# mohammadasim98/mv-ldm

Measured on AMD Instinct MI355X. Metric: denoised views/sec @ 256x256, 4 views, 50 DDIM steps, higher is better.
Workload: dtype bf16

## Files before the change

mv_ldm_amd/_build.py:

```python
from __future__ import annotations

import json
import os
import re
import subprocess
import sys
from concurrent.futures import ThreadPoolExecutor
from pathlib import Path

CSRC = Path(__file__).resolve().parent / "csrc"
LIB = CSRC / "libmvldm_hip.so"
SOURCES = ["api.cpp", "plan.cpp", "igemm.hip", "igemm_small.hip", "igemm_large.hip", "igemm_xl.hip", "igemm_halo.hip", "pack.hip", "attention.hip", "norm.hip", "misc.hip",
           "wgrad.hip", "attention_bwd.hip", "norm_bwd.hip", "train_misc.hip", "linear_pp.hip", "linear_pw.hip", "linear_ws.hip", "linear_rs.hip", "skinny.hip", "metrics.hip"]
HEADERS = [*sorted(CSRC.glob("*.h")), CSRC.parent.parent / "include" / "mvldm.h"]
FLAGS = ["--offload-arch=gfx950", "-O3", "-std=c++17", "-fPIC", "-ffp-contract=off", "-Wno-unused-result",
         "-Rpass-analysis=kernel-resource-usage"]
RES = CSRC / "kernel_resources.json"


def _hipcc() -> str:
    for c in (os.environ.get("HIPCC"), "/opt/rocm/bin/hipcc", "hipcc"):
        if c and (os.path.isabs(c) and os.path.exists(c) or not os.path.isabs(c)):
            return c
    raise RuntimeError("hipcc not found")


def _stale(target: Path, deps) -> bool:
    if not target.exists():
        return True
    t = target.stat().st_mtime
    return any(Path(d).stat().st_mtime > t for d in deps)


def build(force: bool = False, verbose: bool = False) -> Path:
    hipcc = _hipcc()
    flags = list(FLAGS)
    if os.environ.get("MVLDM_EXPERIMENTS") == "1":
        flags.append("-DMVLDM_EXPERIMENTS")
    objs, jobs = [], []
    for src in SOURCES:
        s = CSRC / src
        o = CSRC / (s.stem + ".o")
        objs.append(o)
        if force or _stale(o, [s, *HEADERS]):
            cmd = [hipcc, *flags, "-x", "hip", "-c", str(s), "-o", str(o)]
            jobs.append(cmd)
    if jobs:
        def run(cmd):
            if verbose:
                print(" ".join(cmd), flush=True)
            r = subprocess.run(cmd, capture_output=True, text=True)
            if r.returncode:
                raise RuntimeError(f"hipcc failed: {' '.join(cmd)}\n{r.stdout}\n{r.stderr}")
            Path(cmd[-1]).with_suffix(".res.json").write_text(json.dumps(_resources(r.stderr), indent=0))
        with ThreadPoolExecutor(max_workers=min(8, len(jobs))) as ex:
            list(ex.map(run, jobs))
    if force or jobs or _stale(LIB, objs):
        cmd = [hipcc, "--offload-arch=gfx950", "-shared", "-fPIC", "-o", str(LIB), *map(str, objs)]
        r = subprocess.run(cmd, capture_output=True, text=True)
        if r.returncode:
            raise RuntimeError(f"link failed:\n{r.stdout}\n{r.stderr}")
    parts = [o.with_suffix(".res.json") for o in objs]
    if all(q.exists() for q in parts) and (not RES.exists() or _stale(RES, parts)):
        merged = {}
        for q in parts:
            merged.update(json.loads(q.read_text()))
        RES.write_text(json.dumps(merged, indent=0, sort_keys=True))
    return LIB


_FIELDS = {"VGPRs": "vgpr", "AGPRs": "agpr", "TotalSGPRs": "sgpr", "ScratchSize [bytes/lane]": "scratch", "VGPRs Spill": "vgpr_spill",
           "Occupancy [waves/SIMD]": "waves_per_simd"}


def _resources(stderr: str) -> dict:
    out, cur = {}, None
    for line in stderr.splitlines():
        m = re.search(r"remark:\s+(.*?)\s*\[-Rpass-analysis", line)
        if not m:
            continue
        body = m.group(1)
        if body.startswith("Function Name:"):
            cur = out.setdefault(body.split(":", 1)[1].strip(), {})
        elif cur is not None and ":" in body:
            k, v = body.rsplit(":", 1)
            if k.strip() in _FIELDS and v.strip().lstrip("-").isdigit():
                cur[_FIELDS[k.strip()]] = int(v)
    return out


if __name__ == "__main__":
    print(build(force="--force" in sys.argv, verbose=True))
```

mv_ldm_amd/csrc/attention.hip:

```cpp
#include <algorithm>
#include <cstdlib>

#include "common.h"

namespace mvldm {

struct AttnParams {
    const void* q; const void* k; const void* v; void* out;
    const int32_t* seg;
    int ld_q, ld_k, ld_v, ld_o, heads, d;
    float scale_log2e;
    int nqt;
    int remap;
    float* lse;
    int lse_ld;
};

template <typename T> struct AttnMma;
typedef __attribute__((ext_vector_type(4))) __bf16 bf16x4_t;
typedef __attribute__((ext_vector_type(4))) _Float16 f16x4_t;
template <> struct AttnMma<bf16_t> {
    using Frag = bf16x8;
    using Half = bf16x4_t;
    static __device__ __forceinline__ Half tr_read(const bf16_t* p) {
// ... 258 lines not shown
#pragma unroll
                    for (int r = 0; r < 16; ++r) {
                        const int key = kb * 32 + (r & 3) + 8 * (r >> 2) + 4 * hi;
                        o[0][db] = __builtin_amdgcn_mfma_f32_32x32x2f32(vrow[key], s[0][kb][r], o[0][db], 0, 0, 0);
                    }
            }
        } else {
            const int gi = lane >> 4, sl = lane & 15;
            const T* vsrc = Vt + (4 * (gi >> 1) + (sl >> 2)) * VP + (gi & 1) * 16 + 4 * (sl & 3);
            auto pv = [&](const int qb) {
#pragma unroll
                for (int db = 0; db < NDB; ++db) {
#pragma unroll
                    for (int ks = 0; ks < 4; ++ks) {
                        const T* pa = vsrc + (ks * 16) * VP + db * 32;
                        const auto lo = AttnMma<T>::tr_read(pa);
                        const auto up = AttnMma<T>::tr_read(pa + 8 * VP);
                        const typename AttnMma<T>::Frag a = __builtin_shufflevector(lo, up, 0, 1, 2, 3, 4, 5, 6, 7);
                        o[qb][db] = AttnMma<T>::mma(a, pf[qb][ks], o[qb][db]);
                    }
                }
            };
            if constexpr (QB == 1) {
                sm_max(0);
                sm_exp(0);
                pv(0);
            } else {
                sm_max(0);
                sm_exp(0);
                sm_max(1);
                __builtin_amdgcn_sched_barrier(0);
                pv(0);
                sm_exp(1);
#pragma unroll
                for (int g = 0; g < NDB * 4; ++g) {
                    __builtin_amdgcn_sched_group_barrier(0x100, 2, 0);
                    __builtin_amdgcn_sched_group_barrier(0x008, 1, 0);
                    __builtin_amdgcn_sched_group_barrier(0x002, (96 + NDB * 4 - 1) / (NDB * 4), 0);
                }
                __builtin_amdgcn_sched_barrier(0);
                pv(1);
            }
        }
        __syncthreads();
    }

#pragma unroll
    for (int qb = 0; qb < QB; ++qb) {
        float l_tot;
        if constexpr (ONES) {
            l_tot = 0.f;
#pragma unroll
            for (int db = 0; db < NDB; ++db)
#pragma unroll
                for (int q8 = 0; q8 < 4; ++q8)
                    if (db * 32 + q8 * 8 == d) l_tot = o[qb][db][4 * q8];
        } else {
            l_tot = l_run[qb] + __shfl_xor(l_run[qb], 32, 64);
        }
        const float inv = l_tot > 0.f ? 1.0f / l_tot : 0.f;
        if (!q_ok[qb]) continue;
        if (p.lse && hi == 0) p.lse[(size_t)head * p.lse_ld + q_row0 + q_local[qb]] = m_run[qb] * p.scale_log2e + __log2f(l_tot);
        T* op = reinterpret_cast<T*>(p.out) + (size_t)(q_row0 + q_local[qb]) * p.ld_o + head * d;
#pragma unroll
        for (int db = 0; db < NDB; ++db)
#pragma unroll
            for (int r4 = 0; r4 < 4; ++r4) {
                const int dd = db * 32 + 8 * r4 + 4 * hi;
                if (dd < d) {
                    if constexpr (F32) {
                        f32x4 w = {o[qb][db][r4 * 4 + 0] * inv, o[qb][db][r4 * 4 + 1] * inv, o[qb][db][r4 * 4 + 2] * inv, o[qb][db][r4 * 4 + 3] * inv};
                        *reinterpret_cast<f32x4*>(op + dd) = w;
                    } else {
                        union { T e[4]; u32x2 raw; } w;
#pragma unroll
                        for (int e = 0; e < 4; ++e) w.e[e] = from_f32<T>(o[qb][db][r4 * 4 + e] * inv);
                        *reinterpret_cast<u32x2*>(op + dd) = w.raw;
                    }
                }
            }
    }
}


template <typename T, int NCH>
__global__ __launch_bounds__(256) void attention_wide_kernel(const AttnParams p) {
    constexpr int EPC = Elt<T>::EPC;
    const int lane = threadIdx.x & 63, wave = threadIdx.x >> 6;
    const int head = blockIdx.y;
    const int4 sg = reinterpret_cast<const int4*>(p.seg)[blockIdx.z];
    const int q_row0 = sg.x, q_len = sg.y, kv_row0 = sg.z, kv_len = sg.w;
    const int q_local = blockIdx.x * 4 + wave;
    if (q_local >= q_len) return;
    const int d = p.d, nch = d / EPC;
    const T* qp = reinterpret_cast<const T*>(p.q) + (size_t)(q_row0 + q_local) * p.ld_q + head * d;
    float qv[NCH][EPC], ov[NCH][EPC];
#pragma unroll
    for (int j = 0; j < NCH; ++j) {
        const int ch = lane + 64 * j;
        Chunk<T> c;
        if (ch < nch) c = load_chunk<T>(qp + ch * EPC); else c.zero();
#pragma unroll
        for (int i = 0; i < EPC; ++i) { qv[j][i] = c.get(i) * p.scale_log2e; ov[j][i] = 0.f; }
    }
    const T* kb = reinterpret_cast<const T*>(p.k) + (size_t)kv_row0 * p.ld_k + head * d;
    const T* vb = reinterpret_cast<const T*>(p.v) + (size_t)kv_row0 * p.ld_v + head * d;
    float m_run = -INFINITY, l_run = 0.f;
    for (int key = 0; key < kv_len; ++key) {
        float part = 0.f;
        Chunk<T> vc[NCH];
#pragma unroll
        for (int j = 0; j < NCH; ++j) {
            const int ch = lane + 64 * j;
            Chunk<T> kc;
            if (ch < nch) {
                kc = load_chunk<T>(kb + (size_t)key * p.ld_k + ch * EPC);
                vc[j] = load_chunk<T>(vb + (size_t)key * p.ld_v + ch * EPC);
            } else {
                kc.zero();
                vc[j].zero();
            }
#pragma unroll
            for (int i = 0; i < EPC; ++i) part += qv[j][i] * kc.get(i);
        }
        const float sv = wave_sum(part);
        const float m_new = fmaxf(m_run, sv);
        const float alpha = exp2f(m_run - m_new), pv = exp2f(sv - m_new);
        m_run = m_new;
        l_run = l_run * alpha + pv;
#pragma unroll
        for (int j = 0; j < NCH; ++j)
#pragma unroll
            for (int i = 0; i < EPC; ++i) ov[j][i] = ov[j][i] * alpha + pv * vc[j].get(i);
    }
    const float inv = l_run > 0.f ? 1.0f / l_run : 0.f;
    T* op = reinterpret_cast<T*>(p.out) + (size_t)(q_row0 + q_local) * p.ld_o + head * d;
#pragma unroll
    for (int j = 0; j < NCH; ++j) {
        const int ch = lane + 64 * j;
        if (ch < nch) {
            Chunk<T> c;
#pragma unroll
            for (int i = 0; i < EPC; ++i) c.set(i, ov[j][i] * inv);
            store_chunk<T>(op + ch * EPC, c);
        }
    }
}

constexpr int BKW = 32;
template <typename T, int DSL>
__global__ __launch_bounds__(256, 2)
void attention_dsplit_kernel(const AttnParams p) {
    static_assert(sizeof(T) == 2 && DSL % 32 == 0 && DSL <= 128, "d-split attention: 16-bit, slices of 32..128 columns");
    using Frag = typename AttnMma<T>::Frag;
    constexpr int EPC = 8, D = 4 * DSL;
    constexpr int NDB = DSL / 32, NQ = DSL / 16;
    constexpr int KP = D + 8, VP = v_pitch(D);
    constexpr int NCH = D / EPC;
    constexpr int NST = BKW * NCH / 256;
    static_assert(BKW * NCH % 256 == 0, "whole chunks per thread");
    extern __shared__ __attribute__((aligned(16))) char smem[];
    T* Ks = reinterpret_cast<T*>(smem);
    T* Vt = Ks + BKW * KP;
    float* Xs = reinterpret_cast<float*>(Vt + BKW * VP);

    const int tid = threadIdx.x, lane = tid & 63;
// ... 117 lines not shown
        l_run += rs;
        Frag pf[2];
#pragma unroll
        for (int ks = 0; ks < 2; ++ks)
#pragma unroll
            for (int j = 0; j < 8; ++j) pf[ks][j] = from_f32<T>(s[ks * 8 + j]);
#pragma unroll
        for (int db = 0; db < NDB; ++db)
#pragma unroll
            for (int ks = 0; ks < 2; ++ks) {
                const T* pa = vsrc + (ks * 16) * VP + db * 32;
                const auto lo = AttnMma<T>::tr_read(pa);
                const auto up = AttnMma<T>::tr_read(pa + 8 * VP);
                const Frag a = __builtin_shufflevector(lo, up, 0, 1, 2, 3, 4, 5, 6, 7);
                o[db] = AttnMma<T>::mma(a, pf[ks], o[db]);
            }
        __syncthreads();
    }
    const float l_tot = l_run + __shfl_xor(l_run, 32, 64);
    const float inv = l_tot > 0.f ? 1.0f / l_tot : 0.f;
    if (!q_ok) return;
    T* op = reinterpret_cast<T*>(p.out) + (size_t)(q_row0 + q_local) * p.ld_o + head * D + dsl0;
#pragma unroll
    for (int db = 0; db < NDB; ++db)
#pragma unroll
        for (int r4 = 0; r4 < 4; ++r4) {
            union { T e[4]; u32x2 raw; } w;
#pragma unroll
            for (int e = 0; e < 4; ++e) w.e[e] = from_f32<T>(o[db][r4 * 4 + e] * inv);
            *reinterpret_cast<u32x2*>(op + db * 32 + 8 * r4 + 4 * hi) = w.raw;
        }
}

template <typename T, int DSL> static int launch_attn_dsplit(AttnParams p, int n_seg, int max_q_len, hipStream_t s) {
    constexpr int D = 4 * DSL;
    constexpr int smem = (BKW * (D + 8) + BKW * v_pitch(D)) * 2 + 4 * 64 * 16 * 4;
    auto kern = attention_dsplit_kernel<T, DSL>;
    static std::atomic<uint64_t> attr_done{0};
    if (int rc0 = ensure_dyn_smem(reinterpret_cast<const void*>(kern), smem, attr_done)) return rc0;
    p.nqt = (max_q_len + 31) / 32;
    p.remap = 1;
    hipLaunchKernelGGL(kern, dim3(p.nqt * p.heads * n_seg), dim3(256), smem, s, p);
    return check_launch();
}

template <typename T> static int launch_attn_wide(const AttnParams& p, int n_seg, int max_q_len, hipStream_t s) {
    const int nch = p.d / Elt<T>::EPC;
    dim3 grid((max_q_len + 3) / 4, p.heads, n_seg);
    if (nch <= 64) hipLaunchKernelGGL((attention_wide_kernel<T, 1>), grid, dim3(256), 0, s, p);
    else if (nch <= 128) hipLaunchKernelGGL((attention_wide_kernel<T, 2>), grid, dim3(256), 0, s, p);
    else if (nch <= 256) hipLaunchKernelGGL((attention_wide_kernel<T, 4>), grid, dim3(256), 0, s, p);
    else return set_error(MVLDM_ERR_UNSUPPORTED, "attention: head_dim %d too wide", p.d);
    return check_launch();
}

static const int kEnvAttnQB = knob_int("MVLDM_ATTN_QB", 1);

template <typename T, int DP, bool ONES, int QB> static int launch_attn_k(AttnParams p, int n_seg, int max_q_len, hipStream_t s) {
    constexpr bool F32 = std::is_same<T, float>::value;
    constexpr int DV = (DP + 31) / 32 * 32;
    constexpr int KP = F32 ? (DP + 1) : (DP + 8);
    constexpr int VP = F32 ? (BKV + 1) : v_pitch(DV);
    constexpr int smem = (BKV * KP + (F32 ? DV * VP : BKV * VP)) * (int)sizeof(T);
    auto kern = attention_kernel<T, DP, ONES, QB>;
    static std::atomic<uint64_t> attr_done{0};
    if (int rc0 = ensure_dyn_smem(reinterpret_cast<const void*>(kern), smem, attr_done)) return rc0;
    p.nqt = (max_q_len + BQ * QB - 1) / (BQ * QB);
    p.remap = max_q_len <= 2048;
    dim3 grid(p.nqt * p.heads * n_seg);
    hipLaunchKernelGGL(kern, grid, dim3(256), smem, s, p);
    return check_launch();
}

template <typename T, int DP, bool ONES> static int launch_attn_q(AttnParams p, int n_seg, int max_q_len, hipStream_t s) {
    if constexpr (sizeof(T) == 2 && DP <= 64) {
        const long wgs2 = (long)((max_q_len + 2 * BQ - 1) / (2 * BQ)) * p.heads * n_seg;
        if (kEnvAttnQB == 2 && max_q_len >= 2 * BQ && wgs2 >= 512) return launch_attn_k<T, DP, ONES, 2>(p, n_seg, max_q_len, s);
    }
    return launch_attn_k<T, DP, ONES, 1>(p, n_seg, max_q_len, s);
}

template <typename T, int DP> static int launch_attn(AttnParams p, int n_seg, int max_q_len, hipStream_t s) {
    if constexpr (sizeof(T) == 2) {
        if (p.d % 8 == 0 && p.d < DP) return launch_attn_q<T, DP, true>(p, n_seg, max_q_len, s);
    }
    return launch_attn_q<T, DP, false>(p, n_seg, max_q_len, s);
}

int attention_run(const void* q, const void* k, const void* v, void* out, int ld_q, int ld_k, int ld_v, int ld_o,
                  int heads, int head_dim, const int32_t* seg, int n_seg, int max_q_len, float scale, int dtype,
                  float* lse, int lse_ld, hipStream_t s) {
    const int epc = dtype == MVLDM_F32 ? 4 : 8;
    MVLDM_REQUIRE(head_dim > 0 && head_dim % epc == 0, "attention: head_dim %d must be a multiple of %d", head_dim, epc);
    if (n_seg == 0 || max_q_len == 0) return MVLDM_OK;
    MVLDM_REQUIRE(q && k && v && out && seg, "attention: null pointer");
    MVLDM_REQUIRE(ld_q % epc == 0 && ld_k % epc == 0 && ld_v % epc == 0 && ld_o % 4 == 0, "attention: row strides must keep 16-byte alignment");
    if (n_seg == 0 || max_q_len == 0) return MVLDM_OK;
    MVLDM_REQUIRE(!lse || head_dim <= 160, "attention: log-sum-exp output only on the MFMA kernels (head_dim <= 160)");
    AttnParams p{q, k, v, out, seg, ld_q, ld_k, ld_v, ld_o, heads, head_dim, scale * 1.4426950408889634f, 0, 0, lse, lse_ld};
    const int dp = (head_dim + 15) / 16 * 16;
    return dispatch_dtype(dtype, [&](auto t) {
        using T = decltype(t);
        if (head_dim > 160) {
            if constexpr (sizeof(T) == 2) {
                static const bool valu = knob_int("MVLDM_ATTN_WIDE_VALU", 0) != 0;
                if (head_dim == 512 && !valu && !p.lse) return launch_attn_dsplit<T, 128>(p, n_seg, max_q_len, s);
            }
            return launch_attn_wide<T>(p, n_seg, max_q_len, s);
        }
        switch (dp) {
            case 16: return launch_attn<T, 16>(p, n_seg, max_q_len, s);
            case 32: return launch_attn<T, 32>(p, n_seg, max_q_len, s);
            case 48: return launch_attn<T, 48>(p, n_seg, max_q_len, s);
            case 64: return launch_attn<T, 64>(p, n_seg, max_q_len, s);
            case 80: return launch_attn<T, 80>(p, n_seg, max_q_len, s);
            case 96: return launch_attn<T, 96>(p, n_seg, max_q_len, s);
            case 112: return launch_attn<T, 112>(p, n_seg, max_q_len, s);
            case 128: return launch_attn<T, 128>(p, n_seg, max_q_len, s);
            case 144: return launch_attn<T, 144>(p, n_seg, max_q_len, s);
            case 160: return launch_attn<T, 160>(p, n_seg, max_q_len, s);
            default: return set_error(MVLDM_ERR_UNSUPPORTED, "attention: head_dim %d", head_dim);
        }
    });
}

template <typename T>
__global__ __launch_bounds__(256) void attn_merge_kernel(const T* __restrict__ oa, const float* __restrict__ lse_a, const T* __restrict__ ob,
                                                         const float* __restrict__ lse_b, T* __restrict__ out, const int32_t* __restrict__ a_img,
                                                         const int32_t* __restrict__ b_img, const int32_t* __restrict__ out_img, int n_img, int tokens,
                                                         int heads, int d, int ld_a, int ld_b, int ld_o, int lla, int llb) {
    constexpr int EPC = Elt<T>::EPC;
    const int cpr = heads * d / EPC;
    const size_t total = (size_t)n_img * tokens * cpr;
    for (size_t i = (size_t)blockIdx.x * 256 + threadIdx.x; i < total; i += (size_t)gridDim.x * 256) {
        const int c = (int)(i % cpr);
        const size_t rt = i / cpr;
        const int t = (int)(rt % tokens), k = (int)(rt / tokens);
        const size_t ra = (size_t)a_img[k] * tokens + t, rb = (size_t)b_img[k] * tokens + t, ro = (size_t)out_img[k] * tokens + t;
        const int head = c * EPC / d;
        const float la = lse_a[(size_t)head * lla + ra], lb = lse_b[(size_t)head * llb + rb];
        const float mx = fmaxf(la, lb);
        const float ea = __builtin_amdgcn_exp2f(la - mx), eb = __builtin_amdgcn_exp2f(lb - mx);
        const float inv = 1.0f / (ea + eb);
        const float wa = ea * inv, wb = eb * inv;
        const Chunk<T> va = load_chunk<T>(oa + ra * ld_a + c * EPC), vb = load_chunk<T>(ob + rb * ld_b + c * EPC);
        Chunk<T> o;
#pragma unroll
        for (int e = 0; e < EPC; ++e) o.set(e, va.get(e) * wa + vb.get(e) * wb);
        store_chunk<T>(out + ro * ld_o + c * EPC, o);
    }
}

int attention_merge_run(const void* oa, const float* lse_a, const void* ob, const float* lse_b, void* out, const int32_t* a_img,
                        const int32_t* b_img, const int32_t* out_img, int n_img, int tokens, int heads, int head_dim, int ld_a, int ld_b,
                        int ld_o, int lse_ld_a, int lse_ld_b, int dtype, hipStream_t s) {
    const int epc = dtype == MVLDM_F32 ? 4 : 8;
    if (n_img == 0 || tokens == 0) return MVLDM_OK;
    MVLDM_REQUIRE(oa && ob && out && lse_a && lse_b && a_img && b_img && out_img, "attention_merge: null pointer");
    MVLDM_REQUIRE(head_dim % epc == 0 && ld_a % epc == 0 && ld_b % epc == 0 && ld_o % epc == 0, "attention_merge: 16-byte alignment");
    const size_t total = (size_t)n_img * tokens * (heads * head_dim / epc);
    return dispatch_dtype(dtype, [&](auto t) {
        using T = decltype(t);
        hipLaunchKernelGGL(attn_merge_kernel<T>, dim3((unsigned)std::min<size_t>((total + 255) / 256, 16384)), dim3(256), 0, s, reinterpret_cast<const T*>(oa),
                           lse_a, reinterpret_cast<const T*>(ob), lse_b, reinterpret_cast<T*>(out), a_img, b_img, out_img, n_img, tokens, heads, head_dim,
                           ld_a, ld_b, ld_o, lse_ld_a, lse_ld_b);
        return check_launch();
// ... 18 lines not shown
```

mv_ldm_amd/csrc/igemm.hip:

```cpp
#include <algorithm>
#include <cstdio>
#include <cstdlib>

#include "igemm_common.h"

namespace mvldm {

template <typename T> __global__ __launch_bounds__(256) void igemm_splitk_reduce(const IgemmParams p) {
    const bool geglu = p.epilogue == MVLDM_EPI_GEGLU;
    const size_t total = (size_t)p.M * p.n_dst;
    const size_t slab = (size_t)p.M * p.n_pad;
    for (size_t idx = (size_t)blockIdx.x * 256 + threadIdx.x; idx < total; idx += (size_t)gridDim.x * 256) {
        const int m = (int)(idx / p.n_dst), col = (int)(idx - (size_t)m * p.n_dst);
        float v;
        if (geglu) {
            const int nv = (col >> 5) * 64 + (col & 31), ng = nv + 32;
            float a = 0.f, g = 0.f;
            for (int s = 0; s < p.splitk; ++s) {
                a += p.ws[s * slab + (size_t)m * p.n_pad + nv];
                g += p.ws[s * slab + (size_t)m * p.n_pad + ng];
            }
            if (p.bias) { a += p.bias[col]; g += p.bias[p.n_dst + col]; }
            v = a * gelu_erf_fast(g);
        } else {
// ... 200 lines not shown
        if (!warned) {
            warned = true;
            fprintf(stderr, "[mvldm] igemm: operand of %.2f GB exceeds the 4 GB range of the fast 16-bit loop; using the slower "
                            "64-bit-address loop (split the batch to avoid this)\n", std::max(std::max(b0, b1), bw) / 1e9);
        }
    }
    p.src0_bytes = (unsigned)b0; p.src1_bytes = (unsigned)b1; p.w_bytes = (unsigned)bw;
    p.fake = kEnvFake;
    p.nt_store = stream_stores((size_t)p.M * (size_t)p.n_dst * (p.dst_f32 || d.act_dtype == MVLDM_F32 ? 4 : 2));
    if (kEnvFake & 1) p.src0_bytes = p.src1_bytes = 0;
    if (kEnvFake & 2) p.w_bytes = 0;
    if (tile >= 6 && !p.use_bl) tile = 2;
    if (deep_tile(tile) && d.upsample) tile = 2;
    p.splitk = splitk;
    if (p.use_bl) {
        const int cbs = p.k_tiles / p.taps;
        const int per = cdiv(cbs, std::min(splitk, cbs));
        p.k_tiles_per_split = per * p.taps;
        p.splitk = cdiv(cbs, per);
    } else {
        p.k_tiles_per_split = cdiv(p.k_tiles, splitk);
        p.splitk = cdiv(p.k_tiles, p.k_tiles_per_split);
    }
    p.stage_epi = d.act_dtype != MVLDM_F32 && !kEnvNoStage && (p.splitk > 1 || (!p.dst_f32 && p.n_dst % 8 == 0 && p.dst_ld % 8 == 0));
    if (tile >= 9 && tile <= 10 && (!p.stage_epi || (tile == 10 && d.epilogue == MVLDM_EPI_GEGLU))) tile = 7;
    if (tile == 11 && !(p.use_bl && p.stage_epi && p.splitk == 1 && d.ksize == 3 && d.stride == 1 && d.pad == 1 && !d.upsample &&
                        d.h_out == d.h_in && d.w_out == d.w_in && halo_rows_for(d.w_in) <= 384 && halo_smem(d.w_in) <= 160 * 1024))
        tile = 7;
    if (tile == 17 && !(p.use_bl && p.stage_epi && p.splitk == 1 && d.ksize == 3 && d.stride == 1 && d.pad == 1 && !d.upsample && d.c1 == 0 &&
                        d.h_out == d.h_in && d.w_out == d.w_in && d.epilogue != MVLDM_EPI_GEGLU && halow_smem(d.w_in) <= 160 * 1024))
        tile = 7;
    if (phase) {
        MVLDM_REQUIRE(p.use_bl && p.stage_epi, "igemm: 2x2 phase conv needs the lean 16-bit loop and an 8-aligned 16-bit output");
        if (tile != 7 && tile != 10) tile = 2;
    }
    if (p.use_bl && d.upsample == 1 && tile != 7) tile = 2;
    if (p.use_bl && d.upsample != 1) {
        const int hc = (d.h_out - 1) * d.stride + p.ty0 + p.cy, wc = (d.w_out - 1) * d.stride + p.tx0 + p.cx;
        MVLDM_REQUIRE(p.ty0 + p.cy >= 0 && p.tx0 + p.cx >= 0 && hc < d.h_in && wc < d.w_in,
                      "igemm: conv geometry (pad %d, stride %d) not supported", d.pad, d.stride);
    }
    p.tiles_m = cdiv(p.M, kTiles[tile].bm);
    p.tiles_n = cdiv(d.n_pad, kTiles[tile].bn);
    p.korder = d.k_order;
    if (d.k_order)
        MVLDM_REQUIRE(d.k_order == 1 && p.ctot % bk == 0 && d.c0 % bk == 0 && d.k_pad == p.taps * p.ctot,
                      "igemm: k_order 1 needs channel counts (%d,%d) multiples of %d", d.c0, d.c1, bk);
    {
        const double a_bytes = (double)d.n_img * d.h_in * d.w_in * p.ctot, w_bytes = (double)d.n_pad * d.k_pad;
        double best = 1e300;
        for (int px = 1; px <= 8; px *= 2) {
            const int py = 8 / px;
            const int sm = cdiv(p.tiles_m, px), sn = cdiv(p.tiles_n, py);
            const double waste = (double)(8 * sm * sn) / ((double)p.tiles_m * p.tiles_n);
            const double cost = (py * a_bytes + px * w_bytes) * waste * waste;
            if (cost < best) { best = cost; p.px = px; p.sub_m = sm; p.sub_n = sn; }
        }
        p.m_fast = w_bytes >= a_bytes;
        const int fpx = force_px ? force_px : kEnvPx;
        if (fpx > 0 && fpx <= 8 && (8 % fpx) == 0) {
            p.px = fpx; p.sub_m = cdiv(p.tiles_m, p.px); p.sub_n = cdiv(p.tiles_n, 8 / p.px);
        }
        p.grp_m = p.grp_n = 1;
        static const int kGroup = knob_int("MVLDM_IGEMM_GROUP", -1);
        if (kGroup != 0 && ((tile >= 7 && tile <= 10) || tile == 17) && p.sub_m * p.sub_n > 32) {
            const double ax = a_bytes / p.px, wx = w_bytes / (8 / p.px);
            double bestc = 1e300;
            for (int gm = 1; gm <= 32; gm *= 2) {
                if (kGroup > 0 && gm != kGroup) continue;
                const int gme = std::min(gm, p.sub_m), gne = std::min(32 / gm, p.sub_n);
                const double c = ax * cdiv(p.sub_n, gne) + wx * cdiv(p.sub_m, gme);
                if (c < bestc) { bestc = c; p.grp_m = gme; p.grp_n = gne; }
            }
        }
    }
    return MVLDM_OK;
}

int linear_pp_run(const mvldm_igemm_desc& d, hipStream_t s);
int linear_pw_run(const mvldm_igemm_desc& d, hipStream_t s);
int linear_ws_run(const mvldm_igemm_desc& d, hipStream_t s);
int skinny_run(const mvldm_igemm_desc& d, hipStream_t s);
int linear_rs_run(const mvldm_igemm_desc& d, hipStream_t s);

int igemm_run(const mvldm_igemm_desc& d, hipStream_t s) {
    IgemmParams p;
    int tile = 0;
    if (d.n_img == 0 || d.h_out == 0 || d.w_out == 0) return MVLDM_OK;
    const int req = d.tile & 63;
    if (req == 15) return skinny_run(d, s);
    if (req == 12 || req == 13 || req == 14 || req == 19) {
        MVLDM_REQUIRE(d.src0 && d.weight && d.dst, "igemm: null pointer");
        return req == 12 ? linear_pp_run(d, s) : req == 13 ? linear_pw_run(d, s) : req == 14 ? linear_ws_run(d, s) : linear_rs_run(d, s);
    }
    MVLDM_REQUIRE(d.k_order != 2, "igemm: the fragment-order pack (k_order 2) is read by tile 15 only");
    int rc = fill_params(d, p, tile);
    if (rc) return rc;
    if (p.M == 0) return MVLDM_OK;
    rc = dispatch_dtype(d.act_dtype, [&](auto t) {
        using T = decltype(t);
        int r = launch_igemm(p, tile, Elt<T>::DT, s);
        if (r) return r;
        if (p.splitk > 1) {
            if constexpr (sizeof(T) == 2) {
                if (!p.dst_f32 && p.n_dst % 8 == 0 && p.dst_ld % 8 == 0 && ((uintptr_t)p.ws % 16) == 0 &&
                    (!p.residual || ((uintptr_t)p.residual % 16) == 0) && ((uintptr_t)p.dst % 16) == 0) {
                    const size_t chunks = (size_t)p.M * (p.n_dst / 8);
                    hipLaunchKernelGGL(igemm_splitk_reduce_vec<T>, dim3((unsigned)std::min<size_t>((chunks + 255) / 256, 4096)), dim3(256), 0, s, p);
                    return check_launch();
                }
            }
            const size_t total = (size_t)p.M * p.n_dst;
            const int blocks = (int)std::min<size_t>((total + 255) / 256, 4096);
            hipLaunchKernelGGL(igemm_splitk_reduce<T>, dim3(blocks), dim3(256), 0, s, p);
            return check_launch();
        }
        return (int)MVLDM_OK;
    });
    return rc;
}

}

using namespace mvldm;

extern "C" int mvldm_igemm_fwd(const mvldm_igemm_desc* d, mvldm_stream_t stream) {
    MVLDM_REQUIRE(d != nullptr, "igemm: null desc");
    return igemm_run(*d, (hipStream_t)stream);
}

extern "C" size_t mvldm_igemm_workspace_bytes(const mvldm_igemm_desc* d) {
    if (!d) return 0;
    const size_t M = (size_t)d->n_img * d->h_out * d->w_out;
    return (size_t)16 * M * d->n_pad * sizeof(float);
}
```

mv_ldm_amd/plan.py:

```python
from __future__ import annotations

import ctypes as C
import json
import os
import sys
from dataclasses import dataclass
from typing import List, Optional

import torch

from . import _lib as L
from .ops import PackedWeight, conv_out_hw, dt, igemm_desc, ptr, use_skinny


def _PIN_TILE() -> int:
    v = os.environ.get("MVLDM_IGEMM_TILE")
    return int(v) if v else 0


@dataclass
class OpMeta:
    name: str
    kind: int
    flops: float = 0.0
# ... 413 lines not shown
    return len(_TUNE_CACHE) + len(_WGRAD_CACHE) + len(_SPLIT_CACHE)


def broadcast_tune_cache(dist, src: int = 0, device=None) -> None:
    box = [tune_cache_state() if dist.get_rank() == src else None]
    dist.broadcast_object_list(box, src=src, device=device)
    set_tune_cache_state(box[0], replace=True)


load_tune_cache()


def _igemm_signature(d) -> tuple:
    return (d.n_img, d.h_in, d.w_in, d.h_out, d.w_out, d.c0, d.c1, d.ksize, d.stride, d.pad, d.upsample, d.n_out, d.n_pad,
            d.k_pad, d.epilogue, d.act_dtype, d.dst_dtype, d.k_order, d.dst_ld, bool(d.residual), bool(d.row_bias),
            bool(d.bias), d.splitk, d.workspace_bytes)


_SMALL_ROWS = int(os.environ.get("MVLDM_TUNE_SMALL_ROWS", "64"))
_SPLITS = (0, 1, 2, 4, 8, 16, 32)
_MID_ROWS = int(os.environ.get("MVLDM_TUNE_MID_ROWS", "40000"))
_MID_SPLITS = (0, 1, 2, 3, 4, 6, 8)
_SMALL_TILES = tuple(int(t) for t in os.environ.get("MVLDM_TUNE_SMALL_TILES", "0,1,2,3,4,5").split(","))


_SKINNY = os.environ.get("MVLDM_SKINNY", "1") != "0"
_SKINNY_ROWS = int(os.environ.get("MVLDM_SKINNY_ROWS", "2304"))
_SKINNY_CFGS = tuple(int(c) for c in os.environ.get("MVLDM_SKINNY_CFGS", "0,1,2,5,6,7,8,9,10,12,13,18,19,20,38,39,40,41,42,43,44,46").split(","))


def skinny_rule(rows: int, n_pad: int) -> bool:
    if os.environ.get("MVLDM_AUTOTUNE", "1") != "0" or os.environ.get("MVLDM_SKINNY_RULE", "1") == "0":
        return False
    return rows <= 160 or (rows <= 1152 and n_pad <= 1280)


def skinny_candidate(pw: PackedWeight, rows: int, c0: int, c1: int, upsample, dtype) -> bool:
    return (_SKINNY and dtype != torch.float32 and rows <= _SKINNY_ROWS and not (upsample is True or upsample == 1) and pw.can_skinny()
            and c0 % 64 == 0 and c1 % 64 == 0)


def _unpack_choice(v):
    return (int(v), None) if isinstance(v, int) else (int(v[0]), None if v[1] is None else int(v[1]))


_TUNE_COLD = int(os.environ.get("MVLDM_TUNE_COLD", "9216"))
_THRASH = []
_THRASH_FILLS = [0]


def _thrash(device=None):
    if not _THRASH or (device is not None and _THRASH[0].device != torch.device(device)):
        _THRASH[:] = [torch.empty(640 << 20, dtype=torch.uint8, device=torch.cuda.current_device() if device is None else device)]
    return _THRASH[0]


def autotune_igemm(ops, min_rows: int = 2048, iters: int = 4, srcs=None, skinny=None, keep=None) -> int:
    lib = L.load()
    stream = torch.cuda.current_stream().cuda_stream
    e0, e1 = torch.cuda.Event(enable_timing=True), torch.cuda.Event(enable_timing=True)
    timed = 0
    tune_dev = next((t.device for pair in (srcs or {}).values() for t in pair if t is not None), None)
    if srcs:
        seen, gen = set(), None
        for pair in srcs.values():
            for t in pair:
                if t is not None and t.is_floating_point() and t.data_ptr() not in seen:
                    seen.add(t.data_ptr())
                    if gen is None:
                        gen = torch.Generator(device=t.device)
                        gen.manual_seed(0x5EED)
                    t.normal_(generator=gen)
    for idx, op in enumerate(ops):
        if op.kind != L.OP_IGEMM:
            continue
        d = op.u.igemm
        rows = d.n_img * d.h_out * d.w_out
        sk_pw = (skinny or {}).get(idx)
        if d.tile != 0 or d.act_dtype == L.F32 or d.k_order != 1 or (rows < min(min_rows, _SMALL_ROWS) and sk_pw is None):
            continue
        small = rows < min_rows
        key = _igemm_signature(d) + (("sk",) if sk_pw is not None else ())
        best = _TUNE_CACHE.get(key)
        if best is not None and (_unpack_choice(best)[0] & 63) not in (set(_TUNE_TILES) | set(_SMALL_TILES) | {17, 19} | ({15} if sk_pw is not None else set())):
            best = None
        if best is None:
            trial = L.Op()
            C.memmove(C.byref(trial), C.byref(op), C.sizeof(L.Op))
            can_split = small and bool(d.workspace) and d.splitk == 0
            mid = (not small) and rows < _MID_ROWS and bool(d.workspace) and d.splitk == 0
            cands = [(t, sk) for t in _TUNE_TILES for sk in _MID_SPLITS] if mid else [(t, None) for t in _TUNE_TILES] if not small else \
                    [(t, sk) for t in _SMALL_TILES if t in _TUNE_TILES or not os.environ.get("MVLDM_TUNE_TILES") for sk in (_SPLITS if can_split else (None,))]
            n_it = iters if not small else 3 * iters
            cold = _TUNE_COLD > 0 and rows <= _TUNE_COLD
            if not small and 17 not in _TUNE_TILES and not os.environ.get("MVLDM_TUNE_TILES") and d.ksize == 3 and d.stride == 1 \
                    and d.src1 is None and not d.upsample and d.w_in <= 24:
                cands = cands + [(17, None)]
            if not small and d.ksize == 1 and not os.environ.get("MVLDM_TUNE_TILES"):
                cands = cands + [(19, None), (13 | (1 << 13), None)]
            if sk_pw is not None:
                cands = cands + [(15 | (c << 8), 1) for c in _SKINNY_CFGS]
            results = []
            for tile, sk in cands:
                trial.u.igemm.tile = tile
                trial.u.igemm.splitk = d.splitk if sk is None else sk
                trial.u.igemm.weight, trial.u.igemm.k_order = d.weight, d.k_order
                if (tile & 63) == 15:
                    use_skinny(trial.u.igemm, sk_pw)
                if lib.mvldm_op_run(C.byref(trial), stream) != 0:
                    continue
                if cold:
                    t_sum = 0.0
                    for _ in range(n_it):
                        _thrash(tune_dev).zero_()
                        _THRASH_FILLS[0] += 1
                        e0.record()
                        lib.mvldm_op_run(C.byref(trial), stream)
                        e1.record()
                        e1.synchronize()
                        t_sum += e0.elapsed_time(e1)
                    results.append((t_sum, tile, sk))
                    continue
                e0.record()
                for _ in range(n_it):
                    lib.mvldm_op_run(C.byref(trial), stream)
                e1.record()
                e1.synchronize()
                results.append((e0.elapsed_time(e1), tile, sk))
            t_rule = next(t for t, tile, sk in results if tile == 0 and sk in (None, 0))
            t_best, tile_best, sk_best = min(results, key=lambda r: r[0])
            best = [tile_best, sk_best] if t_best < 0.97 * t_rule else [0, None]
            _TUNE_CACHE[key] = best
            _VALIDATED.add(key)
            timed += 1
        tile, sk = _unpack_choice(best)
        if tile != 0 and key not in _VALIDATED:
            trial = L.Op()
            C.memmove(C.byref(trial), C.byref(op), C.sizeof(L.Op))
            trial.u.igemm.tile = tile
            if sk is not None:
                trial.u.igemm.splitk = sk
            if (tile & 63) == 15:
                if sk_pw is None:
                    tile, sk = 0, None
                else:
                    use_skinny(trial.u.igemm, sk_pw)
            if tile != 0 and lib.mvldm_op_run(C.byref(trial), stream) != 0:
                tile, sk = 0, None
                _TUNE_CACHE[key] = [0, None]
            _VALIDATED.add(key)
        d.tile = tile
        if sk is not None:
            d.splitk = sk
        if (tile & 63) == 15:
            t = use_skinny(d, sk_pw)
            sk_pw._skinny_pinned = True
            if keep is not None:
                keep.append(t)
        elif sk_pw is not None:
            sk_pw.drop_skinny()
    if timed:
        save_tune_cache()
        _THRASH.clear()
    return timed


_BATCH_SPLIT = os.environ.get("MVLDM_BATCH_SPLIT", "1") != "0"
_SPLIT_MIN_ROWS = int(os.environ.get("MVLDM_BATCH_SPLIT_MIN_ROWS", "16384"))


def _split_candidates(d) -> list:
    rpi = d.h_out * d.w_out
    rows = d.n_img * rpi
    out = []
    for bn in (320, 256):
        n_tiles = -(-d.n_pad // bn)
        m_tiles = -(-rows // 256)
        if m_tiles * n_tiles <= 256 or (m_tiles * n_tiles) % 256 == 0 or (m_tiles * n_tiles) % 256 > 216:
            continue
        for m1 in range(m_tiles - 1, 0, -1):
            if (m1 * n_tiles) % 256 == 0 and (m1 * 256) % rpi == 0:
                n1 = m1 * 256 // rpi
# ... 188 lines not shown
```

Baseline: 50.67.

## Add thin-output conv kernel and short-segment attention kernel

Adds a new implicit-GEMM kernel for convolutions with at most 16 output channels. It stages a halo tile and the whole weight in LDS and uses 16x16x32 MFMA, and the autotuner can now pick it as a candidate tile. It also adds a one-wave-per-32-query attention kernel used when the query length is at most 64, which avoids the big-tile flash kernel's waste on short multi-view segments. Both kernels add code paths with narrower support checks and possible LDS occupancy limits.

```diff
diff --git a/mv_ldm_amd/_build.py b/mv_ldm_amd/_build.py
--- a/mv_ldm_amd/_build.py
+++ b/mv_ldm_amd/_build.py
@@ -10,7 +10,7 @@
 
 CSRC = Path(__file__).resolve().parent / "csrc"
 LIB = CSRC / "libmvldm_hip.so"
-SOURCES = ["api.cpp", "plan.cpp", "igemm.hip", "igemm_small.hip", "igemm_large.hip", "igemm_xl.hip", "igemm_halo.hip", "pack.hip", "attention.hip", "norm.hip", "misc.hip",
+SOURCES = ["api.cpp", "plan.cpp", "igemm.hip", "igemm_small.hip", "igemm_large.hip", "igemm_xl.hip", "igemm_halo.hip", "igemm_thin.hip", "pack.hip", "attention.hip", "norm.hip", "misc.hip",
            "wgrad.hip", "attention_bwd.hip", "norm_bwd.hip", "train_misc.hip", "linear_pp.hip", "linear_pw.hip", "linear_ws.hip", "linear_rs.hip", "skinny.hip", "metrics.hip"]
 HEADERS = [*sorted(CSRC.glob("*.h")), CSRC.parent.parent / "include" / "mvldm.h"]
 FLAGS = ["--offload-arch=gfx950", "-O3", "-std=c++17", "-fPIC", "-ffp-contract=off", "-Wno-unused-result",
diff --git a/mv_ldm_amd/csrc/attention.hip b/mv_ldm_amd/csrc/attention.hip
--- a/mv_ldm_amd/csrc/attention.hip
+++ b/mv_ldm_amd/csrc/attention.hip
@@ -364,6 +364,205 @@
     }
 }
 
+constexpr int BKS = 32;
+template <typename T, int DP, bool ONES>
+__global__ __launch_bounds__(256, (DP <= 64 ? 4 : 2))
+void attention_short_kernel(const AttnParams p, const int n_unit) {
+    static_assert(sizeof(T) == 2, "short-segment attention: 16-bit kernels only");
+    using Frag = typename AttnMma<T>::Frag;
+    constexpr int EPC = 8;
+    constexpr int DV = (DP + 31) / 32 * 32, NDB = DV / 32, NQ = DP / 16, NCH = DP / EPC;
+    constexpr int VP = v_pitch(DV);
+    constexpr int NSV = BKS * NCH / 64;
+    extern __shared__ __attribute__((aligned(16))) char smem[];
+    const int lane = threadIdx.x & 63;
+    const int wave = __builtin_amdgcn_readfirstlane(threadIdx.x >> 6);
+    const int hi = lane >> 5, l31 = lane & 31;
+    T* Vt = reinterpret_cast<T*>(smem) + wave * (BKS * VP);
+    const int unit = blockIdx.x * 4 + wave;
+    if (unit >= n_unit) return;
+    const int qb = unit % p.nqt, hs_ = unit / p.nqt;
+    const int head = hs_ % p.heads;
+    const int4 sg = reinterpret_cast<const int4*>(p.seg)[hs_ / p.heads];
+    const int q_row0 = sg.x, q_len = sg.y, kv_row0 = sg.z, kv_len = sg.w;
+    if (qb * 32 >= q_len) return;
+    const int d = p.d;
+
+    const int q_local = qb * 32 + l31;
+    const bool q_ok = q_local < q_len;
+    Frag qf[NQ];
+    {
+        const T* qp = reinterpret_cast<const T*>(p.q) + (size_t)(q_row0 + q_local) * p.ld_q + head * d;
+#pragma unroll
+        for (int kk = 0; kk < NQ; ++kk) {
+            const int dk = kk * 16 + hi * 8;
+            u32x4 raw = u32x4{0u, 0u, 0u, 0u};
+            if (q_ok && dk < d) raw = *reinterpret_cast<const u32x4*>(qp + dk);
+            qf[kk] = __builtin_bit_cast(Frag, raw);
+        }
+    }
+    f32x16 o[NDB];
+#pragma unroll
+    for (int db = 0; db < NDB; ++db)
+#pragma unroll
+        for (int r = 0; r < 16; ++r) o[db][r] = 0.f;
+    float m_run = -INFINITY, l_run = 0.f;
+
+    const char* const kseg = reinterpret_cast<const char*>(reinterpret_cast<const T*>(p.k) + (size_t)kv_row0 * p.ld_k + head * d);
+    const char* const vseg = reinterpret_cast<const char*>(reinterpret_cast<const T*>(p.v) + (size_t)kv_row0 * p.ld_v + head * d);
+    const unsigned kbytes = kv_len > 0 ? ((unsigned)(kv_len - 1) * (unsigned)p.ld_k + (unsigned)d) * 2u : 0u;
+    const unsigned vbytes = kv_len > 0 ? ((unsigned)(kv_len - 1) * (unsigned)p.ld_v + (unsigned)d) * 2u : 0u;
+    const unsigned kstep_bytes = (unsigned)BKS * (unsigned)p.ld_k * 2u, vstep_bytes = (unsigned)BKS * (unsigned)p.ld_v * 2u;
+    const int nstep = (kv_len + BKS - 1) / BKS;
+    const unsigned k_off = ((unsigned)l31 * (unsigned)p.ld_k + (unsigned)(hi * 8)) * 2u;
+    const unsigned k_off_last = ((NQ - 1) * 16 + hi * 8 < d) ? k_off + (unsigned)((NQ - 1) * 32) : kBufOob;
+    unsigned st_vo[NSV], live_bits = 0;
+#pragma unroll
+    for (int j = 0; j < NSV; ++j) {
+        const int idx = lane + 64 * j;
+        const int key = idx / NCH, ch = idx - key * NCH;
+        const bool live = ch * EPC < d;
+        if (live) live_bits |= 1u << j;
+        st_vo[j] = live ? ((unsigned)key * (unsigned)p.ld_v + (unsigned)(ch * EPC)) * 2u : kBufOob;
+        if (!live) {
+            u32x4 zv = u32x4{0u, 0u, 0u, 0u};
+            if constexpr (ONES) {
+                if (ch * EPC == d) {
+                    const uint32_t f = std::is_same<T, bf16_t>::value ? 0x3F803F80u : 0x3C003C00u;
+                    zv = u32x4{f, f, f, f};
+                }
+            }
+            *reinterpret_cast<u32x4*>(Vt + key * VP + ch * EPC) = zv;
+        }
+    }
+    u32x4 rv[NSV];
+    auto load_v = [&](int kt) {
+        const unsigned vo = (unsigned)kt * vstep_bytes;
+#pragma unroll
+        for (int j = 0; j < NSV; ++j) rv[j] = attn_buf_load(vseg + vo, vbytes - vo, st_vo[j]);
+    };
+    if (nstep > 0) load_v(0);
+    const float c = p.scale_log2e;
+    const int gi = lane >> 4, sl = lane & 15;
+    const T* vsrc = Vt + (4 * (gi >> 1) + (sl >> 2)) * VP + (gi & 1) * 16 + 4 * (sl & 3);
+
+    for (int kt = 0; kt < nstep; ++kt) {
+        f32x16 s = f32x16{0.f, 0.f, 0.f, 0.f, 0.f, 0.f, 0.f, 0.f, 0.f, 0.f, 0.f, 0.f, 0.f, 0.f, 0.f, 0.f};
+        {
+            const unsigned ko = (unsigned)kt * kstep_bytes;
+            Frag kf[NQ];
+#pragma unroll
+            for (int kk = 0; kk < NQ; ++kk)
+                kf[kk] = __builtin_bit_cast(Frag, attn_buf_load(kseg + ko, kbytes - ko, kk == NQ - 1 ? k_off_last : k_off + (unsigned)(kk * 32)));
+#pragma unroll
+            for (int kk = 0; kk < NQ; ++kk) s = AttnMma<T>::mma(kf[kk], qf[kk], s);
+        }
+        if (kt == nstep - 1 && (kv_len & (BKS - 1)) != 0) {
+#pragma unroll
+            for (int r = 0; r < 16; ++r) {
+                const int key = kt * BKS + (r & 3) + 8 * (r >> 2) + 4 * hi;
+                s[r] = key < kv_len ? s[r] : -INFINITY;
+            }
+        }
+        float mx = s[0];
+#pragma unroll
+        for (int r = 1; r < 16; ++r) mx = fmaxf(mx, s[r]);
+        mx = fmaxf(mx, __shfl_xor(mx, 32, 64));
+        const float m_new = fmaxf(m_run, mx);
+        const float alpha = __builtin_amdgcn_exp2f((m_run - m_new) * c);
+        m_run = m_new;
+        const float mc = -m_new * c;
+        if constexpr (!ONES) l_run *= alpha;
+        if (!__all(alpha == 1.0f)) {
+#pragma unroll
+            for (int db = 0; db < NDB; ++db)
+#pragma unroll
+                for (int r = 0; r < 16; ++r) o[db][r] *= alpha;
+        }
+        float rs = 0.f;
+#pragma unroll
+        for (int r = 0; r < 16; ++r) {
+            s[r] = __builtin_amdgcn_exp2f(fmaf(s[r], c, mc));
+            if constexpr (!ONES) rs += s[r];
+        }
+        if constexpr (!ONES) l_run += rs;
+        Frag pf[2];
+#pragma unroll
+        for (int ks = 0; ks < 2; ++ks)
+#pragma unroll
+            for (int j = 0; j < 8; ++j) pf[ks][j] = from_f32<T>(s[ks * 8 + j]);
+
+#pragma unroll
+        for (int j = 0; j < NSV; ++j) {
+            if ((live_bits >> j) & 1u) {
+                const int idx = lane + 64 * j;
+                const int key = idx / NCH, ch = idx - key * NCH;
+                *reinterpret_cast<u32x4*>(Vt + key * VP + ch * EPC) = rv[j];
+            }
+        }
+        if (kt + 1 < nstep) load_v(kt + 1);
+        __builtin_amdgcn_fence(__ATOMIC_RELEASE, "wavefront");
+        __builtin_amdgcn_wave_barrier();
+        __builtin_amdgcn_fence(__ATOMIC_ACQUIRE, "wavefront");
+#pragma unroll
+        for (int db = 0; db < NDB; ++db)
+#pragma unroll
+            for (int ks = 0; ks < 2; ++ks) {
+                const T* pa = vsrc + (ks * 16) * VP + db * 32;
+                const auto lo = AttnMma<T>::tr_read(pa);
+                const auto up = AttnMma<T>::tr_read(pa + 8 * VP);
+                const Frag a = __builtin_shufflevector(lo, up, 0, 1, 2, 3, 4, 5, 6, 7);
+                o[db] = AttnMma<T>::mma(a, pf[ks], o[db]);
+            }
+        __builtin_amdgcn_fence(__ATOMIC_RELEASE, "wavefront");
+        __builtin_amdgcn_wave_barrier();
+        __builtin_amdgcn_fence(__ATOMIC_ACQUIRE, "wavefront");
+    }
+
+    float l_tot;
+    if constexpr (ONES) {
+        l_tot = 0.f;
+#pragma unroll
+        for (int db = 0; db < NDB; ++db)
+#pragma unroll
+            for (int q8 = 0; q8 < 4; ++q8)
+                if (db * 32 + q8 * 8 == d) l_tot = o[db][4 * q8];
+    } else {
+        l_tot = l_run + __shfl_xor(l_run, 32, 64);
+    }
+    const float inv = l_tot > 0.f ? 1.0f / l_tot : 0.f;
+    if (!q_ok) return;
+    if (p.lse && hi == 0) p.lse[(size_t)head * p.lse_ld + q_row0 + q_local] = m_run * p.scale_log2e + __log2f(l_tot);
+    T* op = reinterpret_cast<T*>(p.out) + (size_t)(q_row0 + q_local) * p.ld_o + head * d;
+#pragma unroll
+    for (int db = 0; db < NDB; ++db)
+#pragma unroll
+        for (int r4 = 0; r4 < 4; ++r4) {
+            const int dd = db * 32 + 8 * r4 + 4 * hi;
+            if (dd < d) {
+                union { T e[4]; u32x2 raw; } w;
+#pragma unroll
+                for (int e = 0; e < 4; ++e) w.e[e] = from_f32<T>(o[db][r4 * 4 + e] * inv);
+                *reinterpret_cast<u32x2*>(op + dd) = w.raw;
+            }
+        }
+}
+
+template <typename T, int DP> static int launch_attn_short(AttnParams p, int n_seg, int max_q_len, hipStream_t s) {
+    constexpr int DV = (DP + 31) / 32 * 32;
+    constexpr int smem = 4 * BKS * v_pitch(DV) * 2;
+    p.nqt = (max_q_len + 31) / 32;
+    const long n_unit = (long)p.nqt * p.heads * n_seg;
+    MVLDM_REQUIRE(n_unit < (1l << 31), "attention: %ld work units", n_unit);
+    dim3 grid((unsigned)((n_unit + 3) / 4));
+    auto go = [&](auto kern) {
+        hipLaunchKernelGGL(kern, grid, dim3(256), smem, s, p, (int)n_unit);
+        return check_launch();
+    };
+    static_assert(smem <= 48 * 1024, "short-segment attention: four V slices within the default dynamic LDS limit");
+    if (p.d < DP) return go(attention_short_kernel<T, DP, true>);
+    return go(attention_short_kernel<T, DP, false>);
+}
 
 template <typename T, int NCH>
 __global__ __launch_bounds__(256) void attention_wide_kernel(const AttnParams p) {
@@ -647,6 +846,7 @@
 
 template <typename T, int DP> static int launch_attn(AttnParams p, int n_seg, int max_q_len, hipStream_t s) {
     if constexpr (sizeof(T) == 2) {
+        if (max_q_len <= 64) return launch_attn_short<T, DP>(p, n_seg, max_q_len, s);
         if (p.d % 8 == 0 && p.d < DP) return launch_attn_q<T, DP, true>(p, n_seg, max_q_len, s);
     }
     return launch_attn_q<T, DP, false>(p, n_seg, max_q_len, s);
diff --git a/mv_ldm_amd/csrc/igemm.hip b/mv_ldm_amd/csrc/igemm.hip
--- a/mv_ldm_amd/csrc/igemm.hip
+++ b/mv_ldm_amd/csrc/igemm.hip
@@ -306,6 +306,7 @@
 int linear_ws_run(const mvldm_igemm_desc& d, hipStream_t s);
 int skinny_run(const mvldm_igemm_desc& d, hipStream_t s);
 int linear_rs_run(const mvldm_igemm_desc& d, hipStream_t s);
+int igemm_thin_run(const mvldm_igemm_desc& d, hipStream_t s);
 
 int igemm_run(const mvldm_igemm_desc& d, hipStream_t s) {
     IgemmParams p;
@@ -313,6 +314,7 @@
     if (d.n_img == 0 || d.h_out == 0 || d.w_out == 0) return MVLDM_OK;
     const int req = d.tile & 63;
     if (req == 15) return skinny_run(d, s);
+    if (req == 20) return igemm_thin_run(d, s);
     if (req == 12 || req == 13 || req == 14 || req == 19) {
         MVLDM_REQUIRE(d.src0 && d.weight && d.dst, "igemm: null pointer");
         return req == 12 ? linear_pp_run(d, s) : req == 13 ? linear_pw_run(d, s) : req == 14 ? linear_ws_run(d, s) : linear_rs_run(d, s);
diff --git a/mv_ldm_amd/csrc/igemm_thin.hip b/mv_ldm_amd/csrc/igemm_thin.hip
--- /dev/null
+++ b/mv_ldm_amd/csrc/igemm_thin.hip
@@ -0,0 +1,194 @@
+#include "igemm_common.h"
+
+namespace mvldm {
+
+struct ThinParams {
+    const void* src; const void* weight; const float* bias; void* dst;
+    int c0, n_img, h, w, n_out, k_pad, dst_f32, dst_ld, tiles_x, tiles_y, vec_store;
+    unsigned src_bytes;
+};
+
+template <typename T> struct ThinMma;
+template <> struct ThinMma<bf16_t> {
+    using Frag = bf16x8;
+    static __device__ __forceinline__ f32x4 mma(Frag a, Frag b, f32x4 c) { return __builtin_amdgcn_mfma_f32_16x16x32_bf16(a, b, c, 0, 0, 0); }
+};
+template <> struct ThinMma<f16_t> {
+    using Frag = f16x8;
+    static __device__ __forceinline__ f32x4 mma(Frag a, Frag b, f32x4 c) { return __builtin_amdgcn_mfma_f32_16x16x32_f16(a, b, c, 0, 0, 0); }
+};
+
+__device__ __forceinline__ u32x4 thin_buf_load(const void* base, unsigned bytes, unsigned voff) {
+    const __amdgpu_buffer_rsrc_t r = __builtin_amdgcn_make_buffer_rsrc(const_cast<void*>(base), 0, bytes, 0x00020000);
+    return __builtin_amdgcn_raw_buffer_load_b128(r, voff, 0, 0);
+}
+
+constexpr int kThinTile = 16;
+constexpr int kThinPitch = 144;
+inline int thin_w_pitch(int k_pad) { return 2 * k_pad + 16; }
+inline int thin_smem(int ksize, int n_out, int k_pad) {
+    const int hw = kThinTile + 2 * (ksize / 2);
+    return hw * hw * kThinPitch + n_out * thin_w_pitch(k_pad);
+}
+
+template <typename T, int KS>
+__global__ __launch_bounds__(256) void igemm_thin_kernel(const ThinParams p) {
+    using Frag = typename ThinMma<T>::Frag;
+    constexpr int PAD = KS / 2, HS = kThinTile + 2 * PAD, HR = HS * HS, TAPS = KS * KS;
+    constexpr int NCHK = HR * 8;
+    constexpr int NLD = (NCHK + 255) / 256;
+    extern __shared__ __attribute__((aligned(16))) char smem[];
+    char* const halo = smem;
+    char* const wl = smem + HR * kThinPitch;
+    const int wp = 2 * p.k_pad + 16;
+
+    const int tid = threadIdx.x, lane = tid & 63;
+    const int wave = __builtin_amdgcn_readfirstlane(tid >> 6);
+    const int l15 = lane & 15, kg = lane >> 4;
+    const int b = blockIdx.x;
+    const int tx = b % p.tiles_x, ty = (b / p.tiles_x) % p.tiles_y, img = b / (p.tiles_x * p.tiles_y);
+    const int y0 = ty * kThinTile - PAD, x0 = tx * kThinTile - PAD;
+
+    {
+        const int cpr = p.k_pad / 8;
+        const int total = p.n_out * cpr;
+        for (int i = tid; i < total; i += 256) {
+            const int n = i / cpr, c = i - n * cpr;
+            *reinterpret_cast<u32x4*>(wl + n * wp + c * 16) = *reinterpret_cast<const u32x4*>(reinterpret_cast<const char*>(p.weight) + ((size_t)n * p.k_pad + c * 8) * 2);
+        }
+    }
+    unsigned off[NLD], ok_bits = 0;
+#pragma unroll
+    for (int j = 0; j < NLD; ++j) {
+        const int idx = tid + 256 * j;
+        const int r = idx >> 3, ch = idx & 7;
+        const int hy = r / HS, hx = r - hy * HS;
+        const int iy = y0 + hy, ix = x0 + hx;
+        const bool ok = idx < NCHK && (unsigned)iy < (unsigned)p.h && (unsigned)ix < (unsigned)p.w;
+        if (ok) ok_bits |= 1u << j;
+        off[j] = (((unsigned)(img * p.h + iy) * (unsigned)p.w + (unsigned)ix) * (unsigned)p.c0 + (unsigned)(ch * 8)) * 2u;
+    }
+    u32x4 rv[NLD];
+    auto load_halo = [&](int cb) {
+#pragma unroll
+        for (int j = 0; j < NLD; ++j) rv[j] = thin_buf_load(p.src, p.src_bytes, ((ok_bits >> j) & 1u) ? off[j] + (unsigned)(cb * 128) : kBufOob);
+    };
+    auto store_halo = [&]() {
+#pragma unroll
+        for (int j = 0; j < NLD; ++j) {
+            const int idx = tid + 256 * j;
+            if (idx < NCHK) *reinterpret_cast<u32x4*>(halo + (idx >> 3) * kThinPitch + (idx & 7) * 16) = rv[j];
+        }
+    };
+
+    f32x4 acc[4];
+#pragma unroll
+    for (int pb = 0; pb < 4; ++pb) acc[pb] = f32x4{0.f, 0.f, 0.f, 0.f};
+    const int ncb = p.c0 / 64;
+    const bool w_ok = l15 < p.n_out;
+    const char* const wrow = wl + (w_ok ? l15 : 0) * wp + kg * 16;
+    const char* const hrow = halo + ((wave * 4) * HS + l15) * kThinPitch + kg * 16;
+
+    load_halo(0);
+    for (int cb = 0; cb < ncb; ++cb) {
+        __syncthreads();
+        store_halo();
+        if (cb + 1 < ncb) load_halo(cb + 1);
+        __syncthreads();
+#pragma unroll
+        for (int t = 0; t < TAPS; ++t) {
+            const int dy = t / KS, dx = t % KS;
+#pragma unroll
+            for (int ks = 0; ks < 2; ++ks) {
+                u32x4 wraw = u32x4{0u, 0u, 0u, 0u};
+                if (w_ok) wraw = *reinterpret_cast<const u32x4*>(wrow + ((cb * TAPS + t) * 64 + ks * 32) * 2);
+                const Frag a = __builtin_bit_cast(Frag, wraw);
+#pragma unroll
+                for (int pb = 0; pb < 4; ++pb) {
+                    const Frag x = *reinterpret_cast<const Frag*>(hrow + ((pb + dy) * HS + dx) * kThinPitch + ks * 64);
+                    acc[pb] = ThinMma<T>::mma(a, x, acc[pb]);
+                }
+            }
+        }
+    }
+
+    const int n0 = 4 * kg;
+    const int x = tx * kThinTile + l15;
+    if (n0 >= p.n_out || x >= p.w) return;
+    float bv[4];
+#pragma unroll
+    for (int r = 0; r < 4; ++r) bv[r] = (p.bias && n0 + r < p.n_out) ? p.bias[n0 + r] : 0.f;
+#pragma unroll
+    for (int pb = 0; pb < 4; ++pb) {
+        const int y = ty * kThinTile + wave * 4 + pb;
+        if (y >= p.h) continue;
+        const size_t o = ((size_t)(img * p.h + y) * p.w + x) * (size_t)p.dst_ld + n0;
+        if (p.vec_store) {
+            if (p.dst_f32) {
+                *reinterpret_cast<f32x4*>(reinterpret_cast<float*>(p.dst) + o) = f32x4{acc[pb][0] + bv[0], acc[pb][1] + bv[1], acc[pb][2] + bv[2], acc[pb][3] + bv[3]};
+            } else {
+                union { T e[4]; u32x2 raw; } wv;
+#pragma unroll
+                for (int r = 0; r < 4; ++r) wv.e[r] = from_f32<T>(acc[pb][r] + bv[r]);
+                *reinterpret_cast<u32x2*>(reinterpret_cast<T*>(p.dst) + o) = wv.raw;
+            }
+        } else {
+#pragma unroll
+            for (int r = 0; r < 4; ++r) {
+                if (n0 + r < p.n_out) {
+                    if (p.dst_f32) reinterpret_cast<float*>(p.dst)[o + r] = acc[pb][r] + bv[r];
+                    else reinterpret_cast<T*>(p.dst)[o + r] = from_f32<T>(acc[pb][r] + bv[r]);
+                }
+            }
+        }
+    }
+}
+
+template <typename T, int KS> static int launch_thin(const ThinParams& p, int smem, int blocks, hipStream_t s) {
+    static std::atomic<uint64_t> done{0};
+    auto kern = igemm_thin_kernel<T, KS>;
+    if (int rc0 = ensure_dyn_smem(reinterpret_cast<const void*>(kern), 160 * 1024, done)) return rc0;
+    hipLaunchKernelGGL(kern, dim3(blocks), dim3(256), smem, s, p);
+    return check_launch();
+}
+
+int igemm_thin_run(const mvldm_igemm_desc& d, hipStream_t s) {
+    MVLDM_REQUIRE(d.src0 && d.weight && d.dst, "igemm: null pointer");
+    const char* why = nullptr;
+    if (d.act_dtype == MVLDM_F32) why = "16-bit activations only";
+    else if (d.dst_dtype != d.act_dtype && d.dst_dtype != MVLDM_F32) why = "output type";
+    else if (d.k_order != 1) why = "block-major weight pack (k_order 1) only";
+    else if (d.ksize != 1 && d.ksize != 3) why = "1x1 and 3x3 only";
+    else if (d.stride != 1 || d.pad != d.ksize / 2 || d.upsample || d.h_out != d.h_in || d.w_out != d.w_in) why = "stride 1, same-size output only";
+    else if (d.src1 || d.c1) why = "one source only";
+    else if (d.c0 <= 0 || d.c0 % 64 || d.k_pad != d.ksize * d.ksize * d.c0) why = "channels in multiples of 64";
+    else if (d.n_out < 1 || d.n_out > 16 || d.n_pad < d.n_out) why = "at most 16 output channels";
+    else if (d.epilogue != MVLDM_EPI_NONE) why = "no activation epilogue";
+    else if (d.row_bias) why = "no per-image bias row";
+    else if (d.residual) why = "no residual";
+    else if (d.out_scale != 1.0f) why = "no output scale";
+    else if (d.splitk > 1) why = "one K pass only";
+    else if ((double)d.n_img * d.h_in * d.w_in * d.c0 * 2.0 >= 4.0e9) why = "source beyond the 32-bit offset range";
+    else if (thin_smem(d.ksize, d.n_out, d.k_pad) > 160 * 1024) why = "weight does not fit in LDS";
+    else if ((uintptr_t)d.src0 % 16 || (uintptr_t)d.weight % 16) why = "16-byte aligned source and weight";
+    if (why) return set_error(MVLDM_ERR_UNSUPPORTED, "igemm: tile 20 (thin output): %s", why);
+    ThinParams p;
+    p.src = d.src0; p.weight = d.weight; p.bias = d.bias; p.dst = d.dst;
+    p.c0 = d.c0; p.n_img = d.n_img; p.h = d.h_in; p.w = d.w_in; p.n_out = d.n_out; p.k_pad = d.k_pad;
+    p.dst_f32 = d.dst_dtype == MVLDM_F32;
+    p.dst_ld = d.dst_ld > 0 ? d.dst_ld : d.n_out;
+    MVLDM_REQUIRE(p.dst_ld >= d.n_out, "igemm: dst_ld %d < n_dst %d", p.dst_ld, d.n_out);
+    p.tiles_x = cdiv(d.w_in, kThinTile); p.tiles_y = cdiv(d.h_in, kThinTile);
+    p.vec_store = d.n_out % 4 == 0 && p.dst_ld % 4 == 0 && (uintptr_t)d.dst % 16 == 0;
+    p.src_bytes = (unsigned)((size_t)d.n_img * d.h_in * d.w_in * d.c0 * 2);
+    const long blocks = (long)d.n_img * p.tiles_x * p.tiles_y;
+    if (blocks == 0) return MVLDM_OK;
+    if (blocks >= (1l << 31)) return set_error(MVLDM_ERR_UNSUPPORTED, "igemm: tile 20 (thin output): %ld workgroups", blocks);
+    const int smem = thin_smem(d.ksize, d.n_out, d.k_pad);
+    return dispatch_16bit(d.act_dtype, [&](auto t) {
+        using T = decltype(t);
+        return d.ksize == 3 ? launch_thin<T, 3>(p, smem, (int)blocks, s) : launch_thin<T, 1>(p, smem, (int)blocks, s);
+    });
+}
+
+}
diff --git a/mv_ldm_amd/plan.py b/mv_ldm_amd/plan.py
--- a/mv_ldm_amd/plan.py
+++ b/mv_ldm_amd/plan.py
@@ -519,7 +519,7 @@
         small = rows < min_rows
         key = _igemm_signature(d) + (("sk",) if sk_pw is not None else ())
         best = _TUNE_CACHE.get(key)
-        if best is not None and (_unpack_choice(best)[0] & 63) not in (set(_TUNE_TILES) | set(_SMALL_TILES) | {17, 19} | ({15} if sk_pw is not None else set())):
+        if best is not None and (_unpack_choice(best)[0] & 63) not in (set(_TUNE_TILES) | set(_SMALL_TILES) | {17, 19, 20} | ({15} if sk_pw is not None else set())):
             best = None
         if best is None:
             trial = L.Op()
@@ -535,6 +535,8 @@
                 cands = cands + [(17, None)]
             if not small and d.ksize == 1 and not os.environ.get("MVLDM_TUNE_TILES"):
                 cands = cands + [(19, None), (13 | (1 << 13), None)]
+            if d.n_out <= 16 and d.src1 is None and d.stride == 1 and not d.upsample and not os.environ.get("MVLDM_TUNE_TILES"):
+                cands = cands + [(20, None)]
             if sk_pw is not None:
                 cands = cands + [(15 | (c << 8), 1) for c in _SKINNY_CFGS]
             results = []
```

Result: no change. 50.77 (median of 6 runs) (+0.2%).
